# Drexubery/ViewCrafter

Measured on NVIDIA H100. Metric: DDIM denoise-steps/sec @ 576x1024x25f, higher is better.
Workload: dtype f16 (fp32 accumulate; fp32 norms/softmax/update)

## Files before the change

### viewcrafter_b200/csrc/attention.cu

```cuda
#include <cstdlib>

#include "common.cuh"
#include "kernels.h"
#include "wgmma.cuh"

namespace vc {

struct AttnParams {
  CUtensorMap tmap_q, tmap_k, tmap_v;
  __half* out;
  int ldo;
  int Nq, Nk;
  int kv_shared;
  float scale_log2;
  int accumulate;
};

static constexpr int ATT_BM = 128, ATT_D = 64;
static constexpr int ATT_THREADS = 288;
static constexpr int ATT_Q_BYTES = ATT_BM * ATT_D * 2;

template <int BNK>
struct AttnCfg {
  static constexpr int KV_BYTES = BNK * ATT_D * 2;
  static constexpr int SMEM = ATT_Q_BYTES + 4 * KV_BYTES + 1024 + 256;
  static constexpr int MIN_CTAS = BNK == 64 ? 2 : 1;
};

__device__ __forceinline__ float ex2f(float x) {
  float y;
  asm("ex2.approx.ftz.f32 %0, %1;" : "=f"(y) : "f"(x));
  return y;
}

template <int BNK>
__global__ void __launch_bounds__(ATT_THREADS, AttnCfg<BNK>::MIN_CTAS) flash_attn_d64_kernel(const __grid_constant__ AttnParams p) {
  using Cfg = AttnCfg<BNK>;
  extern __shared__ uint8_t smem_raw[];
  uint8_t* smem = reinterpret_cast<uint8_t*>((reinterpret_cast<uintptr_t>(smem_raw) + 1023) & ~uintptr_t(1023));
  uint8_t* sQ = smem;
  uint8_t* sKV = smem + ATT_Q_BYTES;
  uint64_t* bars = reinterpret_cast<uint64_t*>(smem + ATT_Q_BYTES + 4 * Cfg::KV_BYTES);
  uint64_t* q_full = bars + 0;
  uint64_t* kv_full = bars + 1;
  uint64_t* kv_empty = bars + 3;

  const int warp = threadIdx.x >> 5, lane = threadIdx.x & 31;
  const int q0 = blockIdx.x * ATT_BM, head = blockIdx.y, b = blockIdx.z;
  const int bk = p.kv_shared ? 0 : b;
  const int ntiles = (p.Nk + BNK - 1) / BNK;

  if (threadIdx.x == 0) {
    tma_prefetch_desc(&p.tmap_q);
    tma_prefetch_desc(&p.tmap_k);
    tma_prefetch_desc(&p.tmap_v);
    mbar_init(q_full, 1);
    mbar_init(&kv_full[0], 1); mbar_init(&kv_full[1], 1);
    mbar_init(&kv_empty[0], 8); mbar_init(&kv_empty[1], 8);
    fence_barrier_init();
  }
  __syncthreads();

  if (warp == 8) {
    if (elect_one()) {
      mbar_expect_tx(q_full, ATT_Q_BYTES);
      tma_load_4d(sQ, &p.tmap_q, q_full, 0, head, q0, b);
    }
    __syncwarp();
    for (int j = 0; j < ntiles; ++j) {
      const int s = j & 1;
      uint8_t* sk = sKV + s * 2 * Cfg::KV_BYTES;
      if (j >= 2) mbar_wait(&kv_empty[s], ((j >> 1) - 1) & 1);
      if (elect_one()) {
        mbar_expect_tx(&kv_full[s], 2 * Cfg::KV_BYTES);
        tma_load_4d(sk, &p.tmap_k, &kv_full[s], 0, head, j * BNK, bk);
        tma_load_4d(sk + Cfg::KV_BYTES, &p.tmap_v, &kv_full[s], 0, head, j * BNK, bk);
      }
      __syncwarp();
    }
    return;
  }

  const int cw = warp >> 2, wl = warp & 3;
  const uint32_t aQ = smem_u32(sQ) + cw * (64 * ATT_D * 2);
  const float sl2 = p.scale_log2;
  float o[32];
#pragma unroll
  for (int i = 0; i < 32; ++i) o[i] = 0.f;
  float m[2] = {-INFINITY, -INFINITY}, l[2] = {0.f, 0.f};
  mbar_wait(q_full, 0);
  for (int j = 0; j < ntiles; ++j) {
    const int s = j & 1;
    const uint32_t aK = smem_u32(sKV + s * 2 * Cfg::KV_BYTES);
    const uint32_t aV = aK + Cfg::KV_BYTES;
    mbar_wait(&kv_full[s], (j >> 1) & 1);
    float sc[BNK / 2];
    wgmma_fence();
#pragma unroll
    for (int k = 0; k < ATT_D / 16; ++k) Wgmma<BNK>::ss(sc, wgmma_desc_sw128(aQ + 32 * k), wgmma_desc_sw128(aK + 32 * k), k > 0 ? 1 : 0);
    wgmma_commit();
    wgmma_wait<0>();
    wgmma_fence_regs(sc);

    const int valid = p.Nk - j * BNK;
    if (valid < BNK) {
#pragma unroll
      for (int i = 0; i < BNK / 2; ++i) {
        const int col = 8 * (i >> 2) + 2 * (lane & 3) + (i & 1);
        if (col >= valid) sc[i] = -INFINITY;
      }
    }
    float mx[2] = {-INFINITY, -INFINITY};
#pragma unroll
    for (int i = 0; i < BNK / 2; ++i) mx[(i >> 1) & 1] = fmaxf(mx[(i >> 1) & 1], sc[i]);
    float alpha[2], negm[2];
#pragma unroll
    for (int h = 0; h < 2; ++h) {
      mx[h] = fmaxf(mx[h], __shfl_xor_sync(0xffffffffu, mx[h], 1));
      mx[h] = fmaxf(mx[h], __shfl_xor_sync(0xffffffffu, mx[h], 2));
      const float mn = fmaxf(m[h], mx[h] * sl2);
      alpha[h] = ex2f(m[h] - mn);
      m[h] = mn;
      negm[h] = -mn;
      l[h] *= alpha[h];
    }
#pragma unroll
    for (int i = 0; i < 32; ++i) o[i] *= alpha[(i >> 1) & 1];
    uint32_t pa[BNK / 16][4];
#pragma unroll
    for (int kk = 0; kk < BNK / 16; ++kk) {
#pragma unroll
      for (int r = 0; r < 4; ++r) {
        const int i = (2 * kk + (r >> 1)) * 4 + 2 * (r & 1);
        const int h = r & 1;
        const float e0 = ex2f(fmaf(sc[i], sl2, negm[h])), e1 = ex2f(fmaf(sc[i + 1], sl2, negm[h]));
        l[h] += e0 + e1;
        pa[kk][r] = pack_half2(e0, e1);
      }
    }
    wgmma_fence();
#pragma unroll
    for (int kk = 0; kk < BNK / 16; ++kk) Wgmma<64, 1>::rs(o, pa[kk], wgmma_desc_sw128(aV + kk * 16 * 128), 1);
    wgmma_commit();
    wgmma_wait<0>();
    wgmma_fence_regs(o);
    __syncwarp();
    if (lane == 0) mbar_arrive(&kv_empty[s]);
  }

  float inv[2];
#pragma unroll
  for (int h = 0; h < 2; ++h) {
    float t = l[h];
    t += __shfl_xor_sync(0xffffffffu, t, 1);
    t += __shfl_xor_sync(0xffffffffu, t, 2);
    inv[h] = 1.f / t;
  }
#pragma unroll
  for (int h = 0; h < 2; ++h) {
    const int row = q0 + cw * 64 + 16 * wl + (lane >> 2) + 8 * h;
    if (row >= p.Nq) continue;
    __half* op = p.out + ((long long)b * p.Nq + row) * p.ldo + head * ATT_D + 2 * (lane & 3);
#pragma unroll
    for (int jj = 0; jj < 8; ++jj) {
      float v0 = o[jj * 4 + 2 * h] * inv[h], v1 = o[jj * 4 + 2 * h + 1] * inv[h];
      __half2* dst = reinterpret_cast<__half2*>(op + 8 * jj);
      if (p.accumulate) {
        const float2 t = __half22float2(*dst);
        v0 += t.x; v1 += t.y;
      }
      *dst = __floats2half2_rn(v0, v1);
    }
  }
}

static int bn64_mode() {
  static int mode = -2;
  if (mode == -2) { const char* e = getenv("VC_ATTN_BN64"); mode = !e ? -1 : (e[0] == '1' ? 1 : 0); }
  return mode;
}

template <int BNK>
static int launch_attn(const vc_attn_desc& d, cudaStream_t stream) {
  using Cfg = AttnCfg<BNK>;
  AttnParams p;
  memset(&p, 0, sizeof(p));
  {
    uint64_t dims[4] = {64, (uint64_t)d.heads, (uint64_t)d.Nq, (uint64_t)d.B};
    uint64_t str[3] = {128, (uint64_t)d.ldq * 2, (uint64_t)d.ldq * 2 * d.Nq};
    uint32_t box[4] = {64, 1, ATT_BM, 1};
    int rc = encode_tmap_f16(&p.tmap_q, d.q, 4, dims, str, box);
    if (rc) return rc;
  }
  const int shared = d.kv_batch_stride == 0;
  {
    uint64_t dims[4] = {64, (uint64_t)d.heads, (uint64_t)d.Nk, (uint64_t)(shared ? 1 : d.B)};
    uint64_t strk[3] = {128, (uint64_t)d.ldk * 2, (uint64_t)(shared ? (long long)d.ldk * d.Nk : d.kv_batch_stride) * 2};
    uint64_t strv[3] = {128, (uint64_t)d.ldv * 2, (uint64_t)(shared ? (long long)d.ldv * d.Nk : d.kv_batch_stride) * 2};
    uint32_t box[4] = {64, 1, (uint32_t)BNK, 1};
    int rc = encode_tmap_f16(&p.tmap_k, d.k, 4, dims, strk, box);
    if (rc) return rc;
    rc = encode_tmap_f16(&p.tmap_v, d.v, 4, dims, strv, box);
    if (rc) return rc;
  }
  p.out = static_cast<__half*>(d.out); p.ldo = d.ldo; p.Nq = d.Nq; p.Nk = d.Nk; p.kv_shared = shared;
  p.scale_log2 = d.scale * 1.4426950408889634f;
  p.accumulate = d.accumulate;
  static DeviceOnce configured;
  if (device_once_needed(configured)) {
    VC_CHECK_CUDA(cudaFuncSetAttribute(flash_attn_d64_kernel<BNK>, cudaFuncAttributeMaxDynamicSharedMemorySize, Cfg::SMEM));
    device_once_mark(configured);
  }
  dim3 grid((d.Nq + ATT_BM - 1) / ATT_BM, d.heads, d.B);
  flash_attn_d64_kernel<BNK><<<grid, ATT_THREADS, Cfg::SMEM, stream>>>(p);
  VC_CHECK_CUDA(cudaGetLastError());
  return VC_OK;
}

int flash_attn_d64(const vc_attn_desc& d, cudaStream_t stream) {
  VC_REQUIRE(d.q && d.k && d.v && d.out, "flash_attn: null pointer");
  VC_REQUIRE(d.Nq > 0 && d.Nk > 0 && d.B > 0 && d.heads > 0, "flash_attn: empty problem");
  VC_REQUIRE(d.ldq % 8 == 0 && d.ldk % 8 == 0 && d.ldv % 8 == 0 && d.ldo % 8 == 0, "flash_attn: pitches must be multiples of 8");
  VC_REQUIRE(d.kv_batch_stride % 8 == 0, "flash_attn: kv batch stride must be a multiple of 8");
  const int mode = bn64_mode();
  if (mode == 1 || (mode < 0 && d.Nk <= 1024)) return launch_attn<64>(d, stream);
  return launch_attn<128>(d, stream);
}

}
```

Baseline: 2.502.

## Pipeline BNK=128 flash attention with three consumer warpgroups and split K/V stages

For the 128-wide KV tile path, the kernel now runs one producer warpgroup with reduced registers and three MMA warpgroups covering 192 query rows. K and V get separate 3-stage TMA ring buffers. Each consumer issues the next S=QK^T GEMM together with the current PV GEMM, so softmax overlaps tensor-core work. Named-barrier ping-pong orders GEMM issue across warpgroups. This aims to hide softmax latency and raise tensor-core utilisation, at the cost of more register pressure, shared memory and synchronisation complexity.

```diff
diff --git a/viewcrafter_b200/csrc/attention.cu b/viewcrafter_b200/csrc/attention.cu
--- a/viewcrafter_b200/csrc/attention.cu
+++ b/viewcrafter_b200/csrc/attention.cu
@@ -16,14 +16,22 @@
   int accumulate;
 };
 
-static constexpr int ATT_BM = 128, ATT_D = 64;
-static constexpr int ATT_THREADS = 288;
-static constexpr int ATT_Q_BYTES = ATT_BM * ATT_D * 2;
+static constexpr int ATT_D = 64;
+static constexpr int ATT_PRODUCER_REGS = 24;
+static constexpr int ATT_MMA_REGS = 160;
+static_assert(128 * ATT_PRODUCER_REGS + 3 * 128 * ATT_MMA_REGS <= 65536, "register split exceeds the register file");
+static constexpr int ATT_BAR_TURN = 1;
 
 template <int BNK>
 struct AttnCfg {
+  static constexpr bool PIPELINED = BNK == 128;
+  static constexpr int MMA_WGS = PIPELINED ? 3 : 2;
+  static constexpr int BM = 64 * MMA_WGS;
+  static constexpr int Q_BYTES = BM * ATT_D * 2;
+  static constexpr int THREADS = PIPELINED ? 128 * (1 + MMA_WGS) : 288;
+  static constexpr int STAGES = PIPELINED ? 3 : 2;
   static constexpr int KV_BYTES = BNK * ATT_D * 2;
-  static constexpr int SMEM = ATT_Q_BYTES + 4 * KV_BYTES + 1024 + 256;
+  static constexpr int SMEM = Q_BYTES + 2 * STAGES * KV_BYTES + 1024 + 256;
   static constexpr int MIN_CTAS = BNK == 64 ? 2 : 1;
 };
 
@@ -34,120 +42,70 @@
 }
 
 template <int BNK>
-__global__ void __launch_bounds__(ATT_THREADS, AttnCfg<BNK>::MIN_CTAS) flash_attn_d64_kernel(const __grid_constant__ AttnParams p) {
-  using Cfg = AttnCfg<BNK>;
-  extern __shared__ uint8_t smem_raw[];
-  uint8_t* smem = reinterpret_cast<uint8_t*>((reinterpret_cast<uintptr_t>(smem_raw) + 1023) & ~uintptr_t(1023));
-  uint8_t* sQ = smem;
-  uint8_t* sKV = smem + ATT_Q_BYTES;
-  uint64_t* bars = reinterpret_cast<uint64_t*>(smem + ATT_Q_BYTES + 4 * Cfg::KV_BYTES);
-  uint64_t* q_full = bars + 0;
-  uint64_t* kv_full = bars + 1;
-  uint64_t* kv_empty = bars + 3;
-
-  const int warp = threadIdx.x >> 5, lane = threadIdx.x & 31;
-  const int q0 = blockIdx.x * ATT_BM, head = blockIdx.y, b = blockIdx.z;
-  const int bk = p.kv_shared ? 0 : b;
-  const int ntiles = (p.Nk + BNK - 1) / BNK;
-
-  if (threadIdx.x == 0) {
-    tma_prefetch_desc(&p.tmap_q);
-    tma_prefetch_desc(&p.tmap_k);
-    tma_prefetch_desc(&p.tmap_v);
-    mbar_init(q_full, 1);
-    mbar_init(&kv_full[0], 1); mbar_init(&kv_full[1], 1);
-    mbar_init(&kv_empty[0], 8); mbar_init(&kv_empty[1], 8);
-    fence_barrier_init();
-  }
-  __syncthreads();
-
-  if (warp == 8) {
-    if (elect_one()) {
-      mbar_expect_tx(q_full, ATT_Q_BYTES);
-      tma_load_4d(sQ, &p.tmap_q, q_full, 0, head, q0, b);
-    }
-    __syncwarp();
-    for (int j = 0; j < ntiles; ++j) {
-      const int s = j & 1;
-      uint8_t* sk = sKV + s * 2 * Cfg::KV_BYTES;
-      if (j >= 2) mbar_wait(&kv_empty[s], ((j >> 1) - 1) & 1);
-      if (elect_one()) {
-        mbar_expect_tx(&kv_full[s], 2 * Cfg::KV_BYTES);
-        tma_load_4d(sk, &p.tmap_k, &kv_full[s], 0, head, j * BNK, bk);
-        tma_load_4d(sk + Cfg::KV_BYTES, &p.tmap_v, &kv_full[s], 0, head, j * BNK, bk);
-      }
-      __syncwarp();
-    }
-    return;
-  }
-
-  const int cw = warp >> 2, wl = warp & 3;
-  const uint32_t aQ = smem_u32(sQ) + cw * (64 * ATT_D * 2);
-  const float sl2 = p.scale_log2;
-  float o[32];
-#pragma unroll
-  for (int i = 0; i < 32; ++i) o[i] = 0.f;
-  float m[2] = {-INFINITY, -INFINITY}, l[2] = {0.f, 0.f};
-  mbar_wait(q_full, 0);
-  for (int j = 0; j < ntiles; ++j) {
-    const int s = j & 1;
-    const uint32_t aK = smem_u32(sKV + s * 2 * Cfg::KV_BYTES);
-    const uint32_t aV = aK + Cfg::KV_BYTES;
-    mbar_wait(&kv_full[s], (j >> 1) & 1);
-    float sc[BNK / 2];
-    wgmma_fence();
-#pragma unroll
-    for (int k = 0; k < ATT_D / 16; ++k) Wgmma<BNK>::ss(sc, wgmma_desc_sw128(aQ + 32 * k), wgmma_desc_sw128(aK + 32 * k), k > 0 ? 1 : 0);
-    wgmma_commit();
-    wgmma_wait<0>();
-    wgmma_fence_regs(sc);
-
-    const int valid = p.Nk - j * BNK;
-    if (valid < BNK) {
-#pragma unroll
-      for (int i = 0; i < BNK / 2; ++i) {
-        const int col = 8 * (i >> 2) + 2 * (lane & 3) + (i & 1);
-        if (col >= valid) sc[i] = -INFINITY;
-      }
-    }
-    float mx[2] = {-INFINITY, -INFINITY};
-#pragma unroll
-    for (int i = 0; i < BNK / 2; ++i) mx[(i >> 1) & 1] = fmaxf(mx[(i >> 1) & 1], sc[i]);
-    float alpha[2], negm[2];
-#pragma unroll
-    for (int h = 0; h < 2; ++h) {
-      mx[h] = fmaxf(mx[h], __shfl_xor_sync(0xffffffffu, mx[h], 1));
-      mx[h] = fmaxf(mx[h], __shfl_xor_sync(0xffffffffu, mx[h], 2));
-      const float mn = fmaxf(m[h], mx[h] * sl2);
-      alpha[h] = ex2f(m[h] - mn);
-      m[h] = mn;
-      negm[h] = -mn;
-      l[h] *= alpha[h];
-    }
-#pragma unroll
-    for (int i = 0; i < 32; ++i) o[i] *= alpha[(i >> 1) & 1];
-    uint32_t pa[BNK / 16][4];
-#pragma unroll
-    for (int kk = 0; kk < BNK / 16; ++kk) {
-#pragma unroll
-      for (int r = 0; r < 4; ++r) {
-        const int i = (2 * kk + (r >> 1)) * 4 + 2 * (r & 1);
-        const int h = r & 1;
-        const float e0 = ex2f(fmaf(sc[i], sl2, negm[h])), e1 = ex2f(fmaf(sc[i + 1], sl2, negm[h]));
-        l[h] += e0 + e1;
-        pa[kk][r] = pack_half2(e0, e1);
-      }
-    }
-    wgmma_fence();
-#pragma unroll
-    for (int kk = 0; kk < BNK / 16; ++kk) Wgmma<64, 1>::rs(o, pa[kk], wgmma_desc_sw128(aV + kk * 16 * 128), 1);
-    wgmma_commit();
-    wgmma_wait<0>();
-    wgmma_fence_regs(o);
-    __syncwarp();
-    if (lane == 0) mbar_arrive(&kv_empty[s]);
-  }
-
+__device__ __forceinline__ void attn_mask(float (&sc)[BNK / 2], int valid, int lane) {
+#pragma unroll
+  for (int i = 0; i < BNK / 2; ++i) {
+    const int col = 8 * (i >> 2) + 2 * (lane & 3) + (i & 1);
+    if (col >= valid) sc[i] = -INFINITY;
+  }
+}
+
+template <int BNK>
+__device__ __forceinline__ void attn_softmax(const float (&sc)[BNK / 2], float sl2, float (&m)[2], float (&l)[2], float (&alpha)[2],
+                                             float (&e)[BNK / 2]) {
+  constexpr int CH = BNK == 128 ? 4 : 1;
+  float mxc[2][CH];
+#pragma unroll
+  for (int h = 0; h < 2; ++h)
+#pragma unroll
+    for (int c = 0; c < CH; ++c) mxc[h][c] = -INFINITY;
+#pragma unroll
+  for (int i = 0; i < BNK / 2; ++i) mxc[(i >> 1) & 1][(i >> 2) % CH] = fmaxf(mxc[(i >> 1) & 1][(i >> 2) % CH], sc[i]);
+  float mx[2], negm[2];
+#pragma unroll
+  for (int h = 0; h < 2; ++h) {
+    mx[h] = mxc[h][0];
+#pragma unroll
+    for (int c = 1; c < CH; ++c) mx[h] = fmaxf(mx[h], mxc[h][c]);
+    mx[h] = fmaxf(mx[h], __shfl_xor_sync(0xffffffffu, mx[h], 1));
+    mx[h] = fmaxf(mx[h], __shfl_xor_sync(0xffffffffu, mx[h], 2));
+    const float mn = fmaxf(m[h], mx[h] * sl2);
+    alpha[h] = ex2f(m[h] - mn);
+    m[h] = mn;
+    negm[h] = -mn;
+    l[h] *= alpha[h];
+  }
+#pragma unroll
+  for (int kk = 0; kk < BNK / 16; ++kk) {
+#pragma unroll
+    for (int r = 0; r < 4; ++r) {
+      const int i = (2 * kk + (r >> 1)) * 4 + 2 * (r & 1);
+      const int h = r & 1;
+      e[i] = ex2f(fmaf(sc[i], sl2, negm[h]));
+      e[i + 1] = ex2f(fmaf(sc[i + 1], sl2, negm[h]));
+      l[h] += e[i] + e[i + 1];
+    }
+  }
+}
+
+template <int BNK>
+__device__ __forceinline__ void attn_pack(const float (&e)[BNK / 2], uint32_t (&pa)[BNK / 16][4]) {
+#pragma unroll
+  for (int kk = 0; kk < BNK / 16; ++kk)
+#pragma unroll
+    for (int r = 0; r < 4; ++r) {
+      const int i = (2 * kk + (r >> 1)) * 4 + 2 * (r & 1);
+      pa[kk][r] = pack_half2(e[i], e[i + 1]);
+    }
+}
+
+__device__ __forceinline__ void attn_rescale(float (&o)[32], const float (&alpha)[2]) {
+#pragma unroll
+  for (int i = 0; i < 32; ++i) o[i] *= alpha[(i >> 1) & 1];
+}
+
+__device__ __forceinline__ void attn_store(const AttnParams& p, const float (&o)[32], const float (&l)[2], int row0, int wl, int lane,
+                                           int head, int b) {
   float inv[2];
 #pragma unroll
   for (int h = 0; h < 2; ++h) {
@@ -158,7 +116,7 @@
   }
 #pragma unroll
   for (int h = 0; h < 2; ++h) {
-    const int row = q0 + cw * 64 + 16 * wl + (lane >> 2) + 8 * h;
+    const int row = row0 + 16 * wl + (lane >> 2) + 8 * h;
     if (row >= p.Nq) continue;
     __half* op = p.out + ((long long)b * p.Nq + row) * p.ldo + head * ATT_D + 2 * (lane & 3);
 #pragma unroll
@@ -171,6 +129,231 @@
       }
       *dst = __floats2half2_rn(v0, v1);
     }
+  }
+}
+
+template <int BNK>
+__global__ void __launch_bounds__(AttnCfg<BNK>::THREADS, AttnCfg<BNK>::MIN_CTAS) flash_attn_d64_kernel(const __grid_constant__ AttnParams p) {
+  using Cfg = AttnCfg<BNK>;
+  constexpr int STAGES = Cfg::STAGES;
+  extern __shared__ uint8_t smem_raw[];
+  uint8_t* smem = reinterpret_cast<uint8_t*>((reinterpret_cast<uintptr_t>(smem_raw) + 1023) & ~uintptr_t(1023));
+  uint8_t* sQ = smem;
+  uint8_t* sK = smem + Cfg::Q_BYTES;
+  uint8_t* sV = sK + STAGES * Cfg::KV_BYTES;
+  uint64_t* bars = reinterpret_cast<uint64_t*>(sV + STAGES * Cfg::KV_BYTES);
+  uint64_t* q_full = bars + 0;
+  uint64_t* k_full = bars + 1;
+  uint64_t* k_empty = k_full + STAGES;
+  uint64_t* v_full = k_empty + STAGES;
+  uint64_t* v_empty = v_full + STAGES;
+  float* pin = reinterpret_cast<float*>(v_empty + STAGES);
+
+  const int warp = threadIdx.x >> 5, lane = threadIdx.x & 31;
+  const int q0 = blockIdx.x * Cfg::BM, head = blockIdx.y, b = blockIdx.z;
+  const int bk = p.kv_shared ? 0 : b;
+  const int ntiles = (p.Nk + BNK - 1) / BNK;
+  const float sl2 = p.scale_log2;
+
+  if (threadIdx.x == 0) {
+    tma_prefetch_desc(&p.tmap_q);
+    tma_prefetch_desc(&p.tmap_k);
+    tma_prefetch_desc(&p.tmap_v);
+    mbar_init(q_full, 1);
+    for (int s = 0; s < STAGES; ++s) {
+      mbar_init(&k_full[s], 1); mbar_init(&k_empty[s], 4 * Cfg::MMA_WGS);
+      if constexpr (Cfg::PIPELINED) { mbar_init(&v_full[s], 1); mbar_init(&v_empty[s], 4 * Cfg::MMA_WGS); }
+    }
+    fence_barrier_init();
+  }
+  __syncthreads();
+
+  if constexpr (!Cfg::PIPELINED) {
+    if (warp == 8) {
+      if (elect_one()) {
+        mbar_expect_tx(q_full, Cfg::Q_BYTES);
+        tma_load_4d(sQ, &p.tmap_q, q_full, 0, head, q0, b);
+      }
+      __syncwarp();
+      for (int j = 0; j < ntiles; ++j) {
+        const int s = j & 1;
+        if (j >= 2) mbar_wait(&k_empty[s], ((j >> 1) - 1) & 1);
+        if (elect_one()) {
+          mbar_expect_tx(&k_full[s], 2 * Cfg::KV_BYTES);
+          tma_load_4d(sK + s * Cfg::KV_BYTES, &p.tmap_k, &k_full[s], 0, head, j * BNK, bk);
+          tma_load_4d(sV + s * Cfg::KV_BYTES, &p.tmap_v, &k_full[s], 0, head, j * BNK, bk);
+        }
+        __syncwarp();
+      }
+      return;
+    }
+
+    const int cw = warp >> 2, wl = warp & 3;
+    const uint32_t aQ = smem_u32(sQ) + cw * (64 * ATT_D * 2);
+    float o[32];
+#pragma unroll
+    for (int i = 0; i < 32; ++i) o[i] = 0.f;
+    float m[2] = {-INFINITY, -INFINITY}, l[2] = {0.f, 0.f};
+    mbar_wait(q_full, 0);
+    for (int j = 0; j < ntiles; ++j) {
+      const int s = j & 1;
+      const uint32_t aK = smem_u32(sK + s * Cfg::KV_BYTES);
+      const uint32_t aV = smem_u32(sV + s * Cfg::KV_BYTES);
+      mbar_wait(&k_full[s], (j >> 1) & 1);
+      float sc[BNK / 2];
+      wgmma_fence();
+#pragma unroll
+      for (int k = 0; k < ATT_D / 16; ++k) Wgmma<BNK>::ss(sc, wgmma_desc_sw128(aQ + 32 * k), wgmma_desc_sw128(aK + 32 * k), k > 0 ? 1 : 0);
+      wgmma_commit();
+      wgmma_wait<0>();
+      wgmma_fence_regs(sc);
+
+      float alpha[2];
+      float e[BNK / 2];
+      uint32_t pa[BNK / 16][4];
+      if (p.Nk - j * BNK < BNK) attn_mask<BNK>(sc, p.Nk - j * BNK, lane);
+      attn_softmax<BNK>(sc, sl2, m, l, alpha, e);
+      attn_pack<BNK>(e, pa);
+      attn_rescale(o, alpha);
+      wgmma_fence();
+#pragma unroll
+      for (int kk = 0; kk < BNK / 16; ++kk) Wgmma<64, 1>::rs(o, pa[kk], wgmma_desc_sw128(aV + kk * 16 * 128), 1);
+      wgmma_commit();
+      wgmma_wait<0>();
+      wgmma_fence_regs(o);
+      __syncwarp();
+      if (lane == 0) mbar_arrive(&k_empty[s]);
+    }
+    attn_store(p, o, l, q0 + cw * 64, wl, lane, head, b);
+  } else {
+    if (warp < 4) {
+      setmaxnreg_dec<ATT_PRODUCER_REGS>();
+      if (warp != 0) return;
+      if (elect_one()) {
+        mbar_expect_tx(q_full, Cfg::Q_BYTES);
+        tma_load_4d(sQ, &p.tmap_q, q_full, 0, head, q0, b);
+      }
+      __syncwarp();
+      int s = 0, vs = 0;
+      uint32_t ph = 0, vph = 0;
+      for (int j = 0; j <= ntiles; ++j) {
+        if (j < ntiles) {
+          mbar_wait(&k_empty[s], ph ^ 1);
+          if (elect_one()) {
+            mbar_expect_tx(&k_full[s], Cfg::KV_BYTES);
+            tma_load_4d(sK + s * Cfg::KV_BYTES, &p.tmap_k, &k_full[s], 0, head, j * BNK, bk);
+          }
+          __syncwarp();
+          if (++s == STAGES) { s = 0; ph ^= 1; }
+        }
+        if (j > 0) {
+          mbar_wait(&v_empty[vs], vph ^ 1);
+          if (elect_one()) {
+            mbar_expect_tx(&v_full[vs], Cfg::KV_BYTES);
+            tma_load_4d(sV + vs * Cfg::KV_BYTES, &p.tmap_v, &v_full[vs], 0, head, (j - 1) * BNK, bk);
+          }
+          __syncwarp();
+          if (++vs == STAGES) { vs = 0; vph ^= 1; }
+        }
+      }
+      return;
+    }
+
+    setmaxnreg_inc<ATT_MMA_REGS>();
+    const int cw = (warp >> 2) - 1, wl = warp & 3;
+    const uint32_t aQ = smem_u32(sQ) + cw * (64 * ATT_D * 2);
+    const uint32_t aK0 = smem_u32(sK), aV0 = smem_u32(sV);
+    float o[32];
+#pragma unroll
+    for (int i = 0; i < 32; ++i) o[i] = 0.f;
+    float m[2] = {-INFINITY, -INFINITY}, l[2] = {0.f, 0.f};
+    float alpha[2];
+    uint32_t pa[BNK / 16][4];
+    int ks = 0, vs = 0;
+    uint32_t kph = 0, vph = 0;
+
+    constexpr int NWG = Cfg::MMA_WGS;
+    auto turn_wait = [&]() { named_bar_sync(ATT_BAR_TURN + cw, 256); };
+    auto turn_pass = [&](bool last) {
+      if (!(last && cw == NWG - 1)) named_bar_arrive(ATT_BAR_TURN + (cw + 1) % NWG, 256);
+    };
+    auto issue_s = [&](float (&sc)[BNK / 2]) {
+      mbar_wait(&k_full[ks], kph);
+      const uint32_t aK = aK0 + ks * Cfg::KV_BYTES;
+      wgmma_fence();
+#pragma unroll
+      for (int k = 0; k < ATT_D / 16; ++k) Wgmma<BNK>::ss(sc, wgmma_desc_sw128(aQ + 32 * k), wgmma_desc_sw128(aK + 32 * k), k > 0 ? 1 : 0);
+      wgmma_commit();
+    };
+    auto release_k = [&]() {
+      __syncwarp();
+      if (lane == 0) mbar_arrive(&k_empty[ks]);
+      if (++ks == STAGES) { ks = 0; kph ^= 1; }
+    };
+    auto issue_pv = [&]() {
+      mbar_wait(&v_full[vs], vph);
+      const uint32_t aV = aV0 + vs * Cfg::KV_BYTES;
+      wgmma_fence_regs(o);
+      wgmma_fence();
+#pragma unroll
+      for (int kk = 0; kk < BNK / 16; ++kk) Wgmma<64, 1>::rs(o, pa[kk], wgmma_desc_sw128(aV + kk * 16 * 128), 1);
+      wgmma_commit();
+    };
+    auto release_v = [&]() {
+      __syncwarp();
+      if (lane == 0) mbar_arrive(&v_empty[vs]);
+      if (++vs == STAGES) { vs = 0; vph ^= 1; }
+    };
+    auto step = [&](int j, bool partial) {
+      float sc[BNK / 2], e[BNK / 2];
+      turn_wait();
+      issue_s(sc);
+      issue_pv();
+      turn_pass(false);
+      wgmma_wait<1>();
+      wgmma_fence_regs(sc);
+      release_k();
+      if (partial) {
+        wgmma_wait<0>();
+        attn_mask<BNK>(sc, p.Nk - (j + 1) * BNK, lane);
+      }
+      attn_softmax<BNK>(sc, sl2, m, l, alpha, e);
+      if (lane == 0) pin[warp] = l[0] + l[1];
+      wgmma_wait<0>();
+      wgmma_fence_regs(o);
+      release_v();
+      attn_rescale(o, alpha);
+      attn_pack<BNK>(e, pa);
+    };
+
+    mbar_wait(q_full, 0);
+    if (cw == NWG - 1) turn_pass(false);
+    {
+      float sc[BNK / 2], e[BNK / 2];
+      turn_wait();
+      issue_s(sc);
+      turn_pass(false);
+      wgmma_wait<0>();
+      wgmma_fence_regs(sc);
+      release_k();
+      if (p.Nk < BNK) attn_mask<BNK>(sc, p.Nk, lane);
+      attn_softmax<BNK>(sc, sl2, m, l, alpha, e);
+      attn_rescale(o, alpha);
+      attn_pack<BNK>(e, pa);
+    }
+    const bool partial_last = p.Nk % BNK != 0;
+    for (int j = 0; j < ntiles - 2; ++j) step(j, false);
+    if (ntiles >= 2) {
+      if (partial_last) step(ntiles - 2, true);
+      else step(ntiles - 2, false);
+    }
+    turn_wait();
+    issue_pv();
+    turn_pass(true);
+    wgmma_wait<0>();
+    wgmma_fence_regs(o);
+    release_v();
+    attn_store(p, o, l, q0 + cw * 64, wl, lane, head, b);
   }
 }
 
@@ -188,7 +371,7 @@
   {
     uint64_t dims[4] = {64, (uint64_t)d.heads, (uint64_t)d.Nq, (uint64_t)d.B};
     uint64_t str[3] = {128, (uint64_t)d.ldq * 2, (uint64_t)d.ldq * 2 * d.Nq};
-    uint32_t box[4] = {64, 1, ATT_BM, 1};
+    uint32_t box[4] = {64, 1, (uint32_t)Cfg::BM, 1};
     int rc = encode_tmap_f16(&p.tmap_q, d.q, 4, dims, str, box);
     if (rc) return rc;
   }
@@ -211,8 +394,8 @@
     VC_CHECK_CUDA(cudaFuncSetAttribute(flash_attn_d64_kernel<BNK>, cudaFuncAttributeMaxDynamicSharedMemorySize, Cfg::SMEM));
     device_once_mark(configured);
   }
-  dim3 grid((d.Nq + ATT_BM - 1) / ATT_BM, d.heads, d.B);
-  flash_attn_d64_kernel<BNK><<<grid, ATT_THREADS, Cfg::SMEM, stream>>>(p);
+  dim3 grid((d.Nq + Cfg::BM - 1) / Cfg::BM, d.heads, d.B);
+  flash_attn_d64_kernel<BNK><<<grid, Cfg::THREADS, Cfg::SMEM, stream>>>(p);
   VC_CHECK_CUDA(cudaGetLastError());
   return VC_OK;
 }
```

Measured after the change: 2.593 (median of 6 runs). 3.6% higher.
